# zju3dv/SMAP

Measured on NVIDIA H100. Metric: end-to-end FPS @832x512 (backbone+association+lift), higher is better.
Workload: dtype bf16x3 (split-bf16 operands, fp32 accumulate; fp32-faithful)

## Files before the change

### smap_b200/csrc/conv_tc.cuh

```cuda
#pragma once
#include <cuda.h>
#include "common.cuh"

namespace smapb {

struct alignas(64) ConvParams {
    CUtensorMap tmA;
    CUtensorMap tmA2;
    CUtensorMap tmB;
    CUtensorMap tmO;
    CUtensorMap tmR[3];
    int Hout, Wout, Nimg;
    int tw_log2, th;
    int tiles_x, tiles_y;
    int Cout;
    int kh, kw, stride, pad_y, pad_x;
    int kchunks;
    int kchunks2, stride2;
    int n_tiles;
    int total_tiles;
    const float* bias;
    int has_res;
    int n_post;
    __nv_bfloat16* out;
    float* out_f32;
    long long plane_stride;
    int relu;
    int reverse;
    int up_mode, up_Hi, up_Wi, up_pw, up_ph;
    long long* dbg;
    long long* dbg_tl;
    unsigned long long* sat;
};

// ... 196 lines not shown
    const uint32_t ring = (smem_u32(smem_raw) + 1024u + 1023u) & ~1023u;
    const uint32_t out_stage = ring + STAGES * Cfg::STAGE_BYTES;
    const uint32_t res_stage = out_stage + Cfg::OUT_BUFS * Cfg::SLOT_BYTES;

    const int warp = threadIdx.x >> 5;
    const int lane = threadIdx.x & 31;
    const bool tl = p.dbg_tl != nullptr && blockIdx.x == 0;
    if (tl && threadIdx.x == 0) p.dbg_tl[0] = clock64();
    const int n_extra = RING ? p.has_res + p.n_post : 0;
    const bool tma_out = p.out != nullptr;

    if (warp == 0 && lane == 0) {
        tma_prefetch_desc(&p.tmA);
        tma_prefetch_desc(&p.tmB);
        if (p.kchunks2) tma_prefetch_desc(&p.tmA2);
        if (tma_out) tma_prefetch_desc(&p.tmO);
        for (int e = 0; e < n_extra; e++) tma_prefetch_desc(&p.tmR[e]);
    }
    if (warp == 1 && lane == 0) {
        for (int s = 0; s < STAGES; s++) {
            mbar_init(&full_bar[s], 1);
            mbar_init(&empty_bar[s], 4);
        }
        for (int s = 0; s < Cfg::RES_BUFS; s++) {
            mbar_init(&rfull_bar[s], 1);
            mbar_init(&rempty_bar[s], 128);
        }
        fence_mbar_init();
    }
    __syncthreads();

// ... 135 lines not shown
                wgmma_wait<1>();
                if (prev_stage >= 0 && lane == 0) mbar_arrive(&empty_bar[prev_stage]);
                prev_stage = stage;
                if (++stage == STAGES) {
                    stage = 0;
                    phase ^= 1u;
                }
            }
            if (j + 1 < n_cta) turn_pass(TURN_MAIN, wg ^ 1);
            tally(ConvDbg::WAIT_FULL, w_full);
            wgmma_wait<0>();
            if (lane == 0) mbar_arrive(&empty_bar[prev_stage]);
            if (tl && leader && j == n_cta - 1) p.dbg_tl[3] = clock64();

            const long long t_epi0 = timed ? clock64() : 0;
            int py[4], px[4];
            bool valid[4];
            long long pix[4];
#pragma unroll
            for (int q = 0; q < 4; q++) {
                const int row = 64 * (q >> 1) + rw + 8 * (q & 1);
                py[q] = ty * p.th + (row >> p.tw_log2);
                px[q] = (tx << p.tw_log2) + (row & (tw - 1));
                valid[q] = (py[q] < p.Hout) && (px[q] < p.Wout) && (img < p.Nimg);
                pix[q] = ((long long)img * p.Hout + py[q]) * p.Wout + px[q];
            }
            auto row_of = [&](int q) { return 64 * (q >> 1) + rw + 8 * (q & 1); };
            const bool ring_turns = RING != 0 && n_extra > 0;
            if (ring_turns && j > 0) turn_wait(TURN_RING, wg);
            int rcnt = j * Cfg::CHUNKS * n_extra;
            auto ring_wait = [&]() -> uint32_t {
                const int m = rcnt++;
                const int rslot = m % Cfg::RES_DIV;
                tally(ConvDbg::WAIT_RING, mbar_wait_timed(&rfull_bar[rslot], (uint32_t)(m / Cfg::RES_DIV) & 1u, timed));
                return (uint32_t)rslot;
            };
            auto ring_release = [&](uint32_t rslot) {
                fence_proxy_async();
                mbar_arrive(&rempty_bar[rslot]);
            };
// ... 51 lines not shown
                                           (y1i - oy0) * p.up_pw + (x0i - ox0), (y1i - oy0) * p.up_pw + (x1i - ox0)};
#pragma unroll
                        for (int jj = 0; jj < 4; jj++) {
                            float2 s[4];
#pragma unroll
                            for (int k = 0; k < 4; k++) {
                                const uint32_t o = sw64_off(rr[k], jj) + 4 * q4;
                                s[k] = ring_f2(rb, o);
                            }
                            v[q][2 * jj] += hy0 * (wx0 * s[0].x + wx1 * s[1].x) + hy1 * (wx0 * s[2].x + wx1 * s[3].x);
                            v[q][2 * jj + 1] += hy0 * (wx0 * s[0].y + wx1 * s[1].y) + hy1 * (wx0 * s[2].y + wx1 * s[3].y);
                        }
                    }
                    ring_release(rslot);
                }
                if (p.relu) {
#pragma unroll
                    for (int q = 0; q < 4; q++)
#pragma unroll
                        for (int e = 0; e < 8; e++) v[q][e] = fmaxf(v[q][e], 0.f);
                }
                for (int e = 0; RING == 1 && e < p.n_post; e++) ring_add(v);
                if (tma_out) {
                    const uint32_t ob = ob0 + (uint32_t)((((j >> 1) * Cfg::CHUNKS + c) % Cfg::OUT_PER_WG) * Cfg::SLOT_BYTES);
                    if (leader) {
                        const long long t0 = timed ? clock64() : 0;
                        bulk_wait_read<Cfg::OUT_PER_WG - 1>();
                        tally(ConvDbg::WAIT_STAGE, timed ? clock64() - t0 : 0);
                    }
                    bool sat_warp = false;
                    if constexpr (E::F16) {
// ... 22 lines not shown
                                }
                            } else {
                                const uint32_t hw = E::pack2(a, b);
                                sts_u32(ob + o, hw);
                                if (NTERMS == 3)
                                    sts_u32(ob + Cfg::CHUNK_BYTES + o, E::pack2(a - E::lo(hw), b - E::hi(hw)));
                            }
                        }
                    if constexpr (E::F16)
                        if (sat_warp) saturation_add(p.sat, n_sat);
                    fence_proxy_async();
                    epi_bar_sync(wg);
                    if (leader) {
#pragma unroll
                        for (int t = 0; t < Cfg::TA; t++)
                            tma_store_5d(&p.tmO, ob + t * Cfg::CHUNK_BYTES, n0 + c0, tx << p.tw_log2, ty * p.th, img, t);
                        bulk_commit();
                    }
                } else {
#pragma unroll
                    for (int q = 0; q < 4; q++) {
                        if (!valid[q]) continue;
#pragma unroll
                        for (int jj = 0; jj < 4; jj++)
                            *reinterpret_cast<float2*>(p.out_f32 + pix[q] * p.Cout + n0 + c0 + 8 * jj + 2 * q4) =
                                make_float2(v[q][2 * jj], v[q][2 * jj + 1]);
                    }
                }
            }
            if (ring_turns && j + 1 < n_cta) turn_pass(TURN_RING, wg ^ 1);
            tally(ConvDbg::EPILOGUE, timed ? clock64() - t_epi0 : 0);
        }
        if (leader && tma_out) bulk_wait_all();
        if (leader && wg == ((n_cta - 1) & 1)) {
            if (p.dbg) {
                atomicAdd((unsigned long long*)&p.dbg[ConvDbg::TOTAL], (unsigned long long)(clock64() - t_begin));
                atomicAdd((unsigned long long*)&p.dbg[ConvDbg::CTAS], 1ull);
            }
            if (tl) p.dbg_tl[13] = p.dbg_tl[15] = clock64();
        }
// ... 5 lines not shown
```

### smap_b200/csrc/engine.h

```cpp
#pragma once
#include <cuda.h>
#include <cuda_runtime.h>
#include <stdint.h>
#include <stdlib.h>

#include <map>
#include <memory>
#include <string>
#include <vector>

#include "../../include/smap_b200.h"
#include "conv_tc.cuh"
#include "jpeg.h"
#include "png.h"
#include "preprocess.h"
#include "refine.h"

namespace smapb {

struct Act {
    __nv_bfloat16* ptr = nullptr;
    int N = 0, H = 0, W = 0, C = 0;
    long long plane() const { return (long long)N * H * W * C; }
};
struct ActF32 {
    float* ptr = nullptr;
    int N = 0, H = 0, W = 0, C = 0;
};

struct ConvLayer {
    std::string name;
    int Cin = 0, Cout = 0, Cout_pad = 0, k = 1, stride = 1, pad = 0;
    int Cin2 = 0, stride2 = 1;
    __nv_bfloat16* w_dev = nullptr;
    float* bias_dev = nullptr;
};

enum OpKind { OP_STEM, OP_S2D, OP_MAXPOOL, OP_CONV, OP_UPADD, OP_HEADMERGE, OP_TAPSUM };
struct Op {
    OpKind kind;
    ConvParams cp;
    int block_n = 0;
    double flops = 0;
    Act a, b, out;
    ActF32 f4, f3, f2;
    int cout = 0;
    int which_out = 0;
    const float* bias = nullptr;
    int stream = 0;
    std::vector<int> waits;
    bool record = false;
    cudaEvent_t ev = nullptr;
    std::string name;
    std::vector<const void*> inputs;
    int dims[4] = {0, 0, 0, 0};
};

struct Plan {
    int B = 0;
    std::vector<Op> ops;
    std::vector<void*> allocs;
    int n_conv = 0;
    double conv_flops = 0;
    std::map<const void*, int> producer;
    int last_side = -1;
};

}
// ... 145 lines not shown
```

### smap_b200/csrc/plan.cu

```cuda
#include <math.h>
#include <nvtx3/nvToolsExt.h>
#include <stdio.h>
#include <string.h>

#include <algorithm>
#include <mutex>

#include "../../include/smap_b200_debug.h"
#include "elementwise.h"
#include "engine.h"

using namespace smapb;

namespace {

std::mutex g_tiles_mu;
std::map<std::string, std::pair<int, int>> g_tiles;

inline uint16_t f32_to_bf16_rn(float f) {
    uint32_t u;
    memcpy(&u, &f, 4);
    if ((u & 0x7fffffffu) > 0x7f800000u) return (uint16_t)((u >> 16) | 0x40);
    const uint32_t lsb = (u >> 16) & 1u;
    u += 0x7fffu + lsb;
// ... 15 lines not shown
    if (!fn) {
        void* p = nullptr;
        cudaDriverEntryPointQueryResult qres;
        if (cudaGetDriverEntryPoint("cuTensorMapEncodeTiled", &p, cudaEnableDefault, &qres) == cudaSuccess &&
            qres == cudaDriverEntryPointSuccess)
            fn = reinterpret_cast<EncodeTiledFn>(p);
    }
    return fn;
}

struct ConvIO {
    const Act* in = nullptr;
    int relu = 0;
    const Act *in2 = nullptr, *res = nullptr, *post1 = nullptr, *post2 = nullptr, *up = nullptr, *out = nullptr;
    const ActF32* out_f32 = nullptr;
    std::vector<const void*> inputs() const {
        auto p = [](const Act* a) -> const void* { return a ? a->ptr : nullptr; };
        return {in->ptr, p(res), p(post1), p(post2), p(in2), p(up)};
    }
};
const char* const CONV_ROLES[6] = {"in", "res", "p1", "p2", "in2", "up"};

CUtensorMapDataType elem_dtype(const smapb_handle* h) { return h->f16 ? ElemF16::TMA_DTYPE : ElemBF16::TMA_DTYPE; }
int make_act_map(smapb_handle* h, CUtensorMap* m, const __nv_bfloat16* ptr, long long C, long long W, long long H,
                 long long N, int T, long long plane_elems, int box_w, int box_h, int stride, int box_c = 64) {
    EncodeTiledFn fn = get_encode_fn();
    if (!fn) return fail(h, -20, "cuTensorMapEncodeTiled entry point not available");
    cuuint64_t dims[5] = {(cuuint64_t)C, (cuuint64_t)W, (cuuint64_t)H, (cuuint64_t)N, (cuuint64_t)T};
    cuuint64_t strides[4] = {(cuuint64_t)C * 2, (cuuint64_t)W * C * 2, (cuuint64_t)H * W * C * 2,
                             (cuuint64_t)plane_elems * 2};
// ... 94 lines not shown
    return tw;
}

void set_tiling(ConvParams* cp, int nimg, int Hout, int Wout, int tw, int n_tiles) {
    const int th = 128 / tw;
    int twl = 0;
    while ((1 << twl) < tw) twl++;
    cp->Nimg = nimg;
    cp->Hout = Hout;
    cp->Wout = Wout;
    cp->tw_log2 = twl;
    cp->th = th;
    cp->tiles_x = (Wout + tw - 1) / tw;
    cp->tiles_y = (Hout + th - 1) / th;
    cp->n_tiles = n_tiles;
    cp->total_tiles = (int)((long long)cp->tiles_x * cp->tiles_y * nimg * n_tiles);
}

bool is_flat(const ConvLayer& L, const ConvIO& io) {
    return L.k == 1 && L.stride == 1 && (!io.in2 || L.stride2 == 1) && !io.up;
}
void conv_tiling(const ConvLayer& L, const ConvIO& io, int n_tiles, ConvParams* cp) {
    const Act& in = *io.in;
    const int Ho = (in.H + 2 * L.pad - L.k) / L.stride + 1, Wo = (in.W + 2 * L.pad - L.k) / L.stride + 1;
    if (is_flat(L, io))
        set_tiling(cp, 1, 1, (int)((long long)in.N * Ho * Wo), 128, n_tiles);
    else
        set_tiling(cp, in.N, Ho, Wo, patch_width(Ho, Wo, io.in2 ? std::max(L.stride, L.stride2) : L.stride, io.up),
                   n_tiles);
}

int setup_conv(smapb_handle* h, const ConvLayer& L, const ConvIO& io, int block_n, ConvParams* cp) {
    const Act& in = *io.in;
    const Act *in2 = io.in2, *res = io.res, *post1 = io.post1, *post2 = io.post2, *up = io.up;
    if (in.C != L.Cin) return fail(h, -30, "conv " + L.name + ": Cin mismatch");
    if (L.Cin % 64 != 0) return fail(h, -30, "conv " + L.name + ": Cin must be a multiple of 64");
    memset(cp, 0, sizeof(*cp));
    if ((L.Cin2 != 0) != (in2 != nullptr)) return fail(h, -30, "conv " + L.name + ": second input mismatch");
    if (L.Cin2 % 64 != 0) return fail(h, -30, "conv " + L.name + ": Cin2 must be a multiple of 64");
    if (in2 && (in2->C != L.Cin2 || L.k != 1 || L.stride != 1)) return fail(h, -30, "conv " + L.name + ": bad fused pair");
    if (up && (res || post1)) return fail(h, -30, "conv " + L.name + ": up-residual excludes other epilogue inputs");
    const bool flat = is_flat(L, io);
    conv_tiling(L, io, L.Cout_pad / block_n, cp);
    const int N = in.N, tw = 1 << cp->tw_log2, th = cp->th;
    auto a_map = [&](CUtensorMap* m, const Act& a, int s) {
        return flat ? make_act_map(h, m, a.ptr, a.C, cp->Wout, 1, 1, h->planes, a.plane(), 128, 1, 1)
                    : make_act_map(h, m, a.ptr, a.C, a.W, a.H, N, h->planes, a.plane(), tw * s, th * s, s);
    };
    int rc = a_map(&cp->tmA, in, L.stride);
    if (!rc && in2) rc = a_map(&cp->tmA2, *in2, L.stride2);
    if (rc) return rc;
    cp->Cout = L.Cout_pad;
    cp->kh = cp->kw = L.k;
    cp->stride = L.stride;
    cp->pad_y = cp->pad_x = L.pad;
    cp->kchunks = L.Cin / 64;
// ... 5 lines not shown
    if (up) {
        cp->up_mode = 1;
        cp->up_Hi = up->H;
        cp->up_Wi = up->W;
        cp->up_pw = tw / 2 + 2;
        cp->up_ph = th / 2 + 2;
        if (up->H * 2 != cp->Hout || up->W * 2 != cp->Wout || up->C != L.Cout_pad || cp->up_pw * cp->up_ph > 128)
            return fail(h, -30, "conv " + L.name + ": unsupported up-residual geometry");
        rc = make_act_map(h, &cp->tmR[0], up->ptr, up->C, up->W, up->H, N, h->planes, up->plane(), cp->up_pw,
                          cp->up_ph, 1, 32);
        if (rc) return rc;
    }
    if (post2 && !post1) return fail(h, -30, "conv " + L.name + ": post2 without post1");
    cp->out = io.out ? io.out->ptr : nullptr;
    cp->out_f32 = io.out_f32 ? io.out_f32->ptr : nullptr;
    cp->plane_stride = (long long)cp->Nimg * cp->Hout * cp->Wout * L.Cout_pad;
    cp->relu = io.relu;
    cp->sat = h->sat_dev;
    rc = make_w_map(h, &cp->tmB, L.w_dev, L.Cin + L.Cin2, L.Cout_pad, L.k * L.k, h->planes, block_n);
    if (rc) return rc;
    int n_in = up ? 1 : 0;
    for (const Act* t : {io.out, res, post1, post2}) {
        if (!t) continue;
        CUtensorMap* m = t == io.out ? &cp->tmO : &cp->tmR[n_in++];
        rc = make_act_map(h, m, t->ptr, L.Cout_pad, cp->Wout, cp->Hout, cp->Nimg, h->planes, t->plane(), tw, th, 1, 32);
        if (rc) return rc;
    }
    return 0;
}

int setup_stem_conv(smapb_handle* h, const __nv_bfloat16* s2d, long long s2d_plane, int N, int H2, int W2, const Act& out,
                    ConvParams* cp, int* block_n_out, double* flops_out) {
    const ConvLayer& L = h->stem_tc;
    memset(cp, 0, sizeof(*cp));
    EncodeTiledFn fn = get_encode_fn();
    if (!fn) return fail(h, -20, "cuTensorMapEncodeTiled entry point not available");
    set_tiling(cp, N, H2, W2, patch_width(H2, W2, 1, false), 1);
    const long long WP = W2 + 3;
    cuuint64_t dims[5] = {64, (cuuint64_t)W2, (cuuint64_t)H2, (cuuint64_t)N, (cuuint64_t)h->planes};
    cuuint64_t strides[4] = {32, (cuuint64_t)WP * 32, (cuuint64_t)H2 * WP * 32, (cuuint64_t)s2d_plane * 2};
// ... 1 lines not shown
    cuuint32_t es[5] = {1, 1, 1, 1, 1};
    CUresult r = fn(&cp->tmA, elem_dtype(h), 5, (void*)s2d, dims, strides, box, es,
                    CU_TENSOR_MAP_INTERLEAVE_NONE, CU_TENSOR_MAP_SWIZZLE_128B, CU_TENSOR_MAP_L2_PROMOTION_L2_256B,
                    CU_TENSOR_MAP_FLOAT_OOB_FILL_NONE);
    if (r != CUDA_SUCCESS) return fail(h, -22, "sliding-window tensor map rejected: " + std::to_string((int)r));
    cp->Cout = 64;
    cp->kh = 4, cp->kw = 1, cp->stride = 1, cp->pad_y = 2, cp->pad_x = 0;
    cp->kchunks = 1;
    cp->bias = L.bias_dev;
    cp->out = out.ptr;
    cp->plane_stride = out.plane();
    cp->relu = 1;
    cp->sat = h->sat_dev;
    int rc = make_w_map(h, &cp->tmB, L.w_dev, 64, 64, 4, h->planes, 64);
    if (rc) return rc;
    rc = make_act_map(h, &cp->tmO, out.ptr, 64, W2, H2, N, h->planes, out.plane(), 1 << cp->tw_log2, cp->th, 1, 32);
    if (rc) return rc;
    *block_n_out = 64;
    *flops_out = 2.0 * N * H2 * W2 * 64.0 * 147.0;
    return 0;
}

bool table_row_ok(const std::pair<int, int>& row) { return row.second == 1 && tile_shape_ok(row.first); }

int table_tile(smapb_handle* h, const ConvLayer& L, const ConvIO& io, int* bn) {
    const Act& in = *io.in;
    char key[256];
    snprintf(key, sizeof key, "%d/%d/%d k%d s%d %dx%dx%d r%d p%d u%d c2_%d s2_%d t%d%s", L.Cin, L.Cout_pad, L.Cin2, L.k,
             L.stride, in.N, in.H, in.W, io.res ? 1 : 0, (io.post1 ? 1 : 0) + (io.post2 ? 1 : 0), io.up ? 1 : 0, L.Cin2,
             L.stride2, h->nterms, h->f16 ? " f16" : "");
    {
        std::lock_guard<std::mutex> lk(g_tiles_mu);
        auto it = g_tiles.find(key);
        if (it != g_tiles.end() && table_row_ok(it->second)) {
            *bn = it->second.first;
            return 0;
        }
    }
    if (!h->autotune) return 0;
    cudaEvent_t e0, e1;
    cudaEventCreate(&e0);
    cudaEventCreate(&e1);
    float best_ms = 1e30f;
    int best = 0;
    for (int c : {128, 64, 32}) {
        if (L.Cout_pad % c) continue;
        if (c == 32 && L.Cout_pad > 64) continue;
        ConvParams trial;
        if (setup_conv(h, L, io, c, &trial)) continue;
        trial.sat = nullptr;
        float ms_best_c = 1e30f;
        for (int rep = 0; rep < 4; rep++) {
            cudaEventRecord(e0, nullptr);
            if (launch_conv(trial, c, h->nterms, h->f16, h->sm_count, nullptr, false) != cudaSuccess) {
                ms_best_c = 1e30f;
                break;
            }
            cudaEventRecord(e1, nullptr);
            if (cudaEventSynchronize(e1) != cudaSuccess) return fail(h, -10, "autotune launch failed");
            float ms = 0;
            cudaEventElapsedTime(&ms, e0, e1);
            if (rep > 0 && ms < ms_best_c) ms_best_c = ms;
        }
        if (ms_best_c < best_ms) best_ms = ms_best_c, best = c;
    }
    cudaEventDestroy(e0);
    cudaEventDestroy(e1);
    h->err.clear();
    if (!best) return 0;
    std::lock_guard<std::mutex> lk(g_tiles_mu);
    auto it = g_tiles.find(key);
    if (it == g_tiles.end() || !table_row_ok(it->second))
        g_tiles[key] = std::make_pair(best, 1);
    else
        best = it->second.first;
    *bn = best;
    return 0;
}

int choose_tile(smapb_handle* h, const ConvLayer& L, const ConvIO& io, bool tuned, int* bn_out) {
    ConvParams tiling;
    conv_tiling(L, io, 1, &tiling);
    const long long m_tiles = tiling.total_tiles;
    int bn = 0;
    const int num_kb = L.k * L.k * (L.Cin / 64) + L.Cin2 / 64;
    double best = 1e30;
    for (int c : {128, 64, 32}) {
        if (L.Cout_pad % c) continue;
        const double kb_cost = c == 128 ? 1.0 : c == 64 ? 0.6 : 0.4;
        const int n_extra = (io.res || io.up ? 1 : 0) + (io.post1 ? 1 : 0) + (io.post2 ? 1 : 0);
        const double epi = (c / 32) * (0.5 + 0.2 * n_extra + (io.up ? 0.5 : 0.0));
        const long long units = m_tiles * (L.Cout_pad / c);
        const double waves = (double)((units + h->sm_count - 1) / h->sm_count);
        double t = waves * (num_kb * kb_cost + epi);
        t *= (c == 64 ? 1.05 : c == 32 ? 1.10 : 1.0);
        if (t < best - 1e-9) best = t, bn = c;
    }
    if (!bn) return fail(h, -30, "conv " + L.name + ": no tile shape for Cout_pad " + std::to_string(L.Cout_pad));
    if (const char* force = getenv("SMAPB_FORCE_TILE")) {
        int fb = 0;
        if (sscanf(force, "%d", &fb) == 1 && tile_shape_ok(fb) && L.Cout_pad % fb == 0) bn = fb;
    }
    if (tuned) {
        const int rc = table_tile(h, L, io, &bn);
        if (rc) return rc;
    }
    *bn_out = bn;
    return 0;
}

int fold_unit(smapb_handle* h, const std::string& name, std::vector<float>* wf, std::vector<float>* bf, int* Cout,
              int* Cin, int* k) {
    auto need = [&](const char* suffix) -> const std::vector<float>* {
        auto it = h->raw.find(name + suffix);
        return it == h->raw.end() ? nullptr : &it->second;
    };
// ... 46 lines not shown
                if (h->planes == 2) host[plane + o] = f32_to_bf16_rn(v - bf16_to_f32(hi));
            }
    std::vector<float> bias(L.Cout_pad, 0.f);
    for (int co = 0; co < L.Cout; co++) bias[co] = bf[co];
    if (!L.w_dev) {
        if (dev_alloc(h, &L.w_dev, host.size())) return -10;
        if (dev_alloc(h, &L.bias_dev, bias.size())) return -10;
    }
    CK(cudaMemcpy(L.w_dev, host.data(), host.size() * 2, cudaMemcpyHostToDevice));
    CK(cudaMemcpy(L.bias_dev, bias.data(), bias.size() * 4, cudaMemcpyHostToDevice));
    return 0;
}

int pad32(int c) { return (c + 31) / 32 * 32; }

bool precision_ok(int p) { return p == SMAPB_PREC_BF16X3 || p == SMAPB_PREC_BF16 || p == SMAPB_PREC_FP16; }
void set_precision(smapb_handle* h, int precision) {
    h->nterms = precision == SMAPB_PREC_BF16X3 ? 3 : 1;
    h->planes = precision == SMAPB_PREC_BF16X3 ? 2 : 1;
    h->f16 = precision == SMAPB_PREC_FP16;
}

struct PlanBuilder {
    smapb_handle* h;
    Plan* plan;
    int rc = 0;
    int cur_stream = 0;

    void wire(const void* out_ptr, const std::vector<const void*>& inputs) {
        const int idx = (int)plan->ops.size() - 1;
// ... 68 lines not shown
        if (rc) return out;
        Op op;
        op.kind = OP_CONV;
        rc = choose_tile(h, *L, io, !f32, &op.block_n);
        if (!rc) rc = setup_conv(h, *L, io, op.block_n, &op.cp);
        op.flops = 2.0 * in.N * Ho * Wo * (double)L->Cout * (L->Cin * L->k * L->k + L->Cin2);
        op.name = name;
        op.cp.reverse = reverse_for(in.ptr);
        op.dims[0] = in.N, op.dims[1] = Ho, op.dims[2] = Wo, op.dims[3] = L->Cout_pad;
        plan->ops.push_back(op);
        wire(f32 ? (const void*)f32->ptr : out.ptr, io.inputs());
        plan->n_conv++;
        plan->conv_flops += op.flops;
        return out;
    }
};

const void* dumped_output(const smapb_handle* h, const Op& op, long long* bytes) {
    if (op.kind == OP_CONV && op.cp.out) return *bytes = op.cp.plane_stride * h->planes * 2, op.cp.out;
    if (op.kind == OP_CONV && op.cp.out_f32) return *bytes = op.cp.plane_stride * 4, op.cp.out_f32;
    if (op.out.ptr) return *bytes = op.out.plane() * h->planes * 2, op.out.ptr;
    *bytes = 0;
    return nullptr;
}

std::string debug_op_desc(const smapb_handle* h, const Op& op, const std::map<const void*, int>& dump_idx) {
    const bool is_conv = op.kind == OP_CONV;
    const bool stem_tc = is_conv && op.cp.kh == 4 && op.cp.kw == 1;
    const char* kind = is_conv ? (stem_tc ? "stem_tc" : op.cp.out ? "conv" : "conv_f32")
                       : op.kind == OP_STEM ? "stem" : op.kind == OP_S2D ? "s2d" : op.kind == OP_MAXPOOL ? "maxpool"
                       : op.kind == OP_UPADD ? "upadd" : "other";
    std::string s = "name=" + (op.name.empty() ? std::string("?") : op.name) + " kind=" + kind;
    if (op.kind == OP_STEM || op.kind == OP_S2D) s += " in=x";
    for (size_t r = 0; r < op.inputs.size(); r++) {
        if (!op.inputs[r]) continue;
        const char* role = is_conv ? (r < 6 ? CONV_ROLES[r] : "?") : (r == 0 ? "a" : "b");
        auto it = dump_idx.find(op.inputs[r]);
        s += std::string(" ") + role + "=" + (it == dump_idx.end() ? std::string("?") : std::to_string(it->second));
    }
    char buf[320];
    if (is_conv) {
        snprintf(buf, sizeof buf,
                 " tw=%d rev=%d k=%dx%d s=%d pad=%dx%d cin=%d cin2=%d s2=%d cout=%d out=%dx%dx%dx%d bn=%d relu=%d "
                 "hasres=%d post=%d upmode=%d tiles=%d nterms=%d",
                 1 << op.cp.tw_log2, op.cp.reverse, op.cp.kh, op.cp.kw, op.cp.stride, op.cp.pad_y, op.cp.pad_x,
                 op.cp.kchunks * 64, op.cp.kchunks2 * 64, op.cp.stride2, op.cp.Cout, op.dims[0], op.dims[1], op.dims[2],
                 op.dims[3], op.block_n, op.cp.relu, op.cp.has_res, op.cp.n_post, op.cp.up_mode, op.cp.total_tiles,
                 h->nterms);
    } else {
        snprintf(buf, sizeof buf, " out=%dx%dx%dx%d nterms=%d", op.out.N, op.out.H, op.out.W, op.out.C, h->nterms);
    }
    return s + buf + (h->f16 ? " dtype=f16" : "");
}

}

namespace smapb {

void free_plan(Plan* plan) {
    for (void* p : plan->allocs) cudaFree(p);
    for (Op& op : plan->ops)
        if (op.ev) cudaEventDestroy(op.ev);
    plan->allocs.clear();
// ... 65 lines not shown
            pb.wire(stem.ptr, {});
        }
    }
    Act x = pb.new_act(B, H / 4, W / 4, 64);
    {
        Op op;
        op.kind = OP_MAXPOOL;
        op.name = "top.maxpool";
        op.a = stem;
        op.out = x;
        plan->ops.push_back(op);
        pb.wire(x.ptr, {stem.ptr});
    }
    Act skip1[4], skip2[4];
    ActF32 res[4], resd3, resrd3;
    std::string name_d, name_rd;
    for (int s = 0; s < 3 && !pb.rc; s++) {
        const std::string pre = "stage" + std::to_string(s) + ".";
        const bool gen_skip = s != 2;
        Act feats[4];
        Act t = x;
        for (int li = 0; li < 4; li++) {
            for (int b = 0; b < LAYERS[li]; b++) {
                const std::string p = pre + "downsample.layer" + std::to_string(li + 1) + "." + std::to_string(b) + ".";
                Act o1 = pb.conv(p + "conv_bn_relu1", {&t, 1});
                Act o2 = pb.conv(p + "conv_bn_relu2", {&o1, 1});
                const bool last = (b == LAYERS[li] - 1) && s > 0;
                ConvIO c3{&o2, 1};
                if (b == 0 && !getenv("SMAPB_NO_FUSE_DS")) {
                    c3.in2 = &t;
                    t = pb.conv(p + "fused_conv3_downsample", c3);
                } else if (b == 0) {
                    Act idn = pb.conv(p + "downsample", {&t, 0});
                    c3.res = &idn;
                    t = pb.conv(p + "conv_bn_relu3", c3);
                } else {
                    c3.res = &t;
                    if (last) c3.post1 = &skip1[li], c3.post2 = &skip2[li];
                    t = pb.conv(p + "conv_bn_relu3", c3);
                }
            }
            feats[li] = t;
        }
        Act up_x;
        Act sk1[4], sk2[4];
        Act cross;
        for (int ind = 0; ind < 4 && !pb.rc; ind++) {
            const std::string p = pre + "upsample.up" + std::to_string(ind + 1) + ".";
            const Act& xin = feats[3 - ind];
            Act out;
            if (ind == 0) {
                out = pb.conv(p + "u_skip", {&xin, 1});
            } else {
                Act tl = pb.conv(p + "up_conv", {&up_x, 0});
                if (!getenv("SMAPB_NO_FUSE_UP")) {
                    ConvIO io{&xin, 1};
                    io.up = &tl;
                    out = pb.conv(p + "u_skip", io);
                } else {
                    Act a = pb.conv(p + "u_skip", {&xin, 0});
                    out = pb.new_act(a.N, a.H, a.W, a.C);
                    Op op;
                    op.kind = OP_UPADD;
                    op.a = a;
                    op.b = tl;
                    op.out = out;
                    plan->ops.push_back(op);
                    pb.wire(out.ptr, {a.ptr, tl.ptr});
                }
            }
            pb.cur_stream = h->two_streams ? 1 : 0;
            if (s == 2 && ind >= 1) {
                Act r1 = pb.conv(p + "res_conv1", {&out, 1});
                pb.conv(p + "res_conv2", {&r1, 0}, &res[ind]);
            }
            if (s == 2 && ind == 3) {
                Act d1 = pb.conv(p + "res_d_conv1", {&out, 1});
                pb.conv(p + "res_d_conv2.tapexp", {&d1, 0}, &resd3);
                Act rd1 = pb.conv(p + "res_rd_conv1", {&out, 1});
                pb.conv(p + "res_rd_conv2.tapexp", {&rd1, 0}, &resrd3);
                name_d = p + "res_d_conv2";
                name_rd = p + "res_rd_conv2";
            }
            if (gen_skip) {
                sk1[ind] = pb.conv(p + "skip1", {&xin, 1});
                sk2[ind] = pb.conv(p + "skip2", {&out, 1});
                pb.cur_stream = 0;
                if (ind == 3) cross = pb.conv(p + "cross_conv", {&out, 1});
            }
            pb.cur_stream = 0;
            up_x = out;
        }
        for (int li = 0; li < 4; li++) {
            skip1[li] = sk1[3 - li];
            skip2[li] = sk2[3 - li];
        }
        x = cross;
    }
    if (pb.rc) {
        free_plan(plan.get());
        return pb.rc;
    }
    {
// ... 117 lines not shown
        cudaDeviceSynchronize();
        for (auto& kv : h->plans) free_plan(kv.second.get());
        h->plans.clear();
        free_layers(h);
    }
    set_precision(h, precision);
    std::vector<std::string> units;
    for (auto& kv : h->raw) {
        const std::string& k = kv.first;
        const std::string suf = ".conv.weight";
        if (k.size() > suf.size() && k.compare(k.size() - suf.size(), suf.size(), suf) == 0)
            units.push_back(k.substr(0, k.size() - suf.size()));
    }
    if (units.empty()) return fail(h, -40, "no weights loaded");
    std::map<std::string, std::pair<std::vector<float>, std::vector<float>>> folded;
    for (const std::string& name : units) {
        std::vector<float> wf, bf;
        int Cout, Cin, k;
        int rc = fold_unit(h, name, &wf, &bf, &Cout, &Cin, &k);
        if (rc) return rc;
        if (name.find(".downsample.layer") != std::string::npos &&
            (name.find(".0.conv_bn_relu3") != std::string::npos ||
             (name.size() > 13 && name.compare(name.size() - 13, 13, ".0.downsample") == 0)))
            folded[name] = {wf, bf};
        if (name.find("res_d_conv2") != std::string::npos || name.find("res_rd_conv2") != std::string::npos)
            folded[name] = {wf, bf};
        if (name == "top.conv") {
            if (Cin != 3 || Cout != 64 || k != 7) return fail(h, -40, "top.conv must be 3->64 7x7");
            std::vector<float> w2(147 * 64);
            for (int co = 0; co < 64; co++)
                for (int ci = 0; ci < 3; ci++)
                    for (int ky = 0; ky < 7; ky++)
                        for (int kx = 0; kx < 7; kx++)
                            w2[((ky * 7 + kx) * 3 + ci) * 64 + co] = wf[((co * 3 + ci) * 7 + ky) * 7 + kx];
            if (!h->stem_w) {
// ... 78 lines not shown
        if (L0.k != 3) continue;
        ConvLayer& E = h->layers[nm + ".tapexp"];
        E.name = nm + ".tapexp";
        E.Cin = L0.Cin;
        E.Cout = 9 * L0.Cout;
        E.Cout_pad = pad32(E.Cout);
        E.k = 1, E.stride = 1, E.pad = 0;
        std::vector<float> wf((size_t)E.Cout * E.Cin), bf(E.Cout, 0.f);
        for (int c = 0; c < L0.Cout; c++)
            for (int ci = 0; ci < L0.Cin; ci++)
                for (int t = 0; t < 9; t++)
                    wf[(size_t)(t * L0.Cout + c) * E.Cin + ci] = kv.second.first[((size_t)c * L0.Cin + ci) * 9 + t];
        int rc4 = upload_conv_layer(h, E, 1, wf, bf);
        if (rc4) return rc4;
    }
    if (!h->stem_w) return fail(h, -40, "top.conv weights missing");
    h->finalized = true;
    return 0;
}

int smapb_set_tile_table(const char* text) {
    if (!text) return -1;
    std::lock_guard<std::mutex> lk(g_tiles_mu);
    int n = 0;
    const char* p = text;
    while (*p) {
        const char* e = strchr(p, '\n');
        std::string line = e ? std::string(p, e - p) : std::string(p);
        p = e ? e + 1 : p + line.size();
        if (line.empty() || line[0] == '#') continue;
// ... 21 lines not shown

__global__ void checksum_kernel(const uint32_t* __restrict__ p, long long nwords, unsigned long long* out) {
    unsigned long long acc = 0;
    for (long long i = (long long)blockIdx.x * blockDim.x + threadIdx.x; i < nwords; i += (long long)gridDim.x * blockDim.x)
        acc += (unsigned long long)p[i] * (unsigned long long)((i % 1021) + 1);
    atomicAdd(out, acc);
}
long long smapb_debug_dump(smapb_handle* h, int B, int idx, void* host, long long max_bytes, int which) {
    if (!h) return -1;
    cudaSetDevice(h->device);
    Plan* plan = nullptr;
    int rc = build_plan(h, B, &plan);
    if (rc) return rc;
    cudaDeviceSynchronize();
    int n = 0;
    for (const Op& op : plan->ops) {
        long long bytes = 0;
        const void* ptr = dumped_output(h, op, &bytes);
        if (!ptr) continue;
        if (n++ != idx) continue;
        (void)which;
        if (bytes > max_bytes) bytes = max_bytes;
        if (bytes > 0) CK(cudaMemcpy(host, ptr, (size_t)bytes, cudaMemcpyDefault));
        return bytes;
    }
    return -2;
}

int smapb_debug_checksums(smapb_handle* h, int B, unsigned long long* sums, int max_ops, char* desc, int desc_stride) {
    if (!h) return -1;
    cudaSetDevice(h->device);
    Plan* plan = nullptr;
    int rc = build_plan(h, B, &plan);
    if (rc) return rc;
    CK(cudaDeviceSynchronize());
    unsigned long long* d = nullptr;
    CK(cudaMalloc((void**)&d, 8));
    std::map<const void*, int> dump_idx;
    int n_dumped = 0;
    for (const Op& op : plan->ops) {
        long long bytes = 0;
        const void* out = dumped_output(h, op, &bytes);
        if (!out) continue;
        if (!dump_idx.emplace(out, n_dumped++).second) {
            cudaFree(d);
            return fail(h, -2, "smapb_debug_checksums: two ops share an output tensor (" + op.name + ")");
        }
    }
    int n = 0;
    for (const Op& op : plan->ops) {
        if (n >= max_ops) break;
        long long bytes = 0;
        const void* ptr = dumped_output(h, op, &bytes);
        if (!ptr) continue;
        const long long words = bytes / 4;
        CK(cudaMemset(d, 0, 8));
        checksum_kernel<<<132 * 4, 256>>>((const uint32_t*)ptr, words, d);
        CK(cudaMemcpy(&sums[n], d, 8, cudaMemcpyDeviceToHost));
        if (desc) snprintf(desc + (size_t)n * desc_stride, desc_stride, "%s", debug_op_desc(h, op, dump_idx).c_str());
        n++;
    }
    cudaFree(d);
    return n;
}

int smapb_plan_info(const smapb_handle* hc, int B, int* n_conv, double* conv_flops) {
    smapb_handle* h = const_cast<smapb_handle*>(hc);
    if (!h) return -1;
    if (!h->finalized) return fail(h, -2, "weights not finalized");
    cudaSetDevice(h->device);
    Plan* plan = nullptr;
    int rc = build_plan(h, B, &plan);
    if (rc) return rc;
    if (n_conv) *n_conv = plan->n_conv;
    if (conv_flops) *conv_flops = plan->conv_flops;
    return 0;
// ... 198 lines not shown
```

Before: 480.0.

## Merge sibling 1x1 convs sharing an input into one multi-output GEMM

Concatenates the weights of sibling 1x1 convolutions that read the same activation (skip2+up_conv, res_conv1+up_conv, the three res conv1 branches) into one merged layer. The kernel picks a per-segment output tensor map and relu bit from the N-tile index, so one launch writes several separate outputs. This cuts kernel launches and re-reads of the shared input, and gives each launch more N-tiles to fill the GPU. In exchange it adds per-segment bookkeeping in the epilogue, requires the block width to divide every segment, and restructures stream placement and the debug dump paths.

```diff
diff --git a/smap_b200/csrc/conv_tc.cuh b/smap_b200/csrc/conv_tc.cuh
--- a/smap_b200/csrc/conv_tc.cuh
+++ b/smap_b200/csrc/conv_tc.cuh
@@ -3,12 +3,14 @@
 #include "common.cuh"
 
 namespace smapb {
+
+constexpr int SEG_MAX = 3;
 
 struct alignas(64) ConvParams {
     CUtensorMap tmA;
     CUtensorMap tmA2;
     CUtensorMap tmB;
-    CUtensorMap tmO;
+    CUtensorMap tmO[SEG_MAX];
     CUtensorMap tmR[3];
     int Hout, Wout, Nimg;
     int tw_log2, th;
@@ -18,6 +20,7 @@
     int kchunks;
     int kchunks2, stride2;
     int n_tiles;
+    int seg_nt[SEG_MAX];
     int total_tiles;
     const float* bias;
     int has_res;
@@ -244,7 +247,8 @@
         tma_prefetch_desc(&p.tmA);
         tma_prefetch_desc(&p.tmB);
         if (p.kchunks2) tma_prefetch_desc(&p.tmA2);
-        if (tma_out) tma_prefetch_desc(&p.tmO);
+        if (tma_out) tma_prefetch_desc(&p.tmO[0]);
+        for (int s = 1; RING == 0 && s < SEG_MAX && p.seg_nt[s] < p.n_tiles; s++) tma_prefetch_desc(&p.tmO[s]);
         for (int e = 0; e < n_extra; e++) tma_prefetch_desc(&p.tmR[e]);
     }
     if (warp == 1 && lane == 0) {
@@ -410,16 +414,16 @@
             if (tl && leader && j == n_cta - 1) p.dbg_tl[3] = clock64();
 
             const long long t_epi0 = timed ? clock64() : 0;
+            const int seg = RING ? 0 : (n0 >= p.seg_nt[1] * BLOCK_N) + (n0 >= p.seg_nt[2] * BLOCK_N);
+            const int n0_out = RING ? n0 : n0 - p.seg_nt[seg] * BLOCK_N;
             int py[4], px[4];
             bool valid[4];
-            long long pix[4];
 #pragma unroll
             for (int q = 0; q < 4; q++) {
                 const int row = 64 * (q >> 1) + rw + 8 * (q & 1);
                 py[q] = ty * p.th + (row >> p.tw_log2);
                 px[q] = (tx << p.tw_log2) + (row & (tw - 1));
                 valid[q] = (py[q] < p.Hout) && (px[q] < p.Wout) && (img < p.Nimg);
-                pix[q] = ((long long)img * p.Hout + py[q]) * p.Wout + px[q];
             }
             auto row_of = [&](int q) { return 64 * (q >> 1) + rw + 8 * (q & 1); };
             const bool ring_turns = RING != 0 && n_extra > 0;
@@ -501,7 +505,7 @@
                     }
                     ring_release(rslot);
                 }
-                if (p.relu) {
+                if (RING ? p.relu : (p.relu >> seg) & 1) {
 #pragma unroll
                     for (int q = 0; q < 4; q++)
 #pragma unroll
@@ -554,16 +558,18 @@
                     if (leader) {
 #pragma unroll
                         for (int t = 0; t < Cfg::TA; t++)
-                            tma_store_5d(&p.tmO, ob + t * Cfg::CHUNK_BYTES, n0 + c0, tx << p.tw_log2, ty * p.th, img, t);
+                            tma_store_5d(&p.tmO[seg], ob + t * Cfg::CHUNK_BYTES, n0_out + c0, tx << p.tw_log2, ty * p.th,
+                                         img, t);
                         bulk_commit();
                     }
                 } else {
 #pragma unroll
                     for (int q = 0; q < 4; q++) {
                         if (!valid[q]) continue;
+                        const long long pix = ((long long)img * p.Hout + py[q]) * p.Wout + px[q];
 #pragma unroll
                         for (int jj = 0; jj < 4; jj++)
-                            *reinterpret_cast<float2*>(p.out_f32 + pix[q] * p.Cout + n0 + c0 + 8 * jj + 2 * q4) =
+                            *reinterpret_cast<float2*>(p.out_f32 + pix * p.Cout + n0 + c0 + 8 * jj + 2 * q4) =
                                 make_float2(v[q][2 * jj], v[q][2 * jj + 1]);
                     }
                 }
diff --git a/smap_b200/csrc/engine.h b/smap_b200/csrc/engine.h
--- a/smap_b200/csrc/engine.h
+++ b/smap_b200/csrc/engine.h
@@ -28,10 +28,16 @@
     int N = 0, H = 0, W = 0, C = 0;
 };
 
+struct ConvSeg {
+    std::string name;
+    int Cout = 0, Cout_pad = 0;
+};
+
 struct ConvLayer {
     std::string name;
     int Cin = 0, Cout = 0, Cout_pad = 0, k = 1, stride = 1, pad = 0;
     int Cin2 = 0, stride2 = 1;
+    std::vector<ConvSeg> segs;
     __nv_bfloat16* w_dev = nullptr;
     float* bias_dev = nullptr;
 };
@@ -52,6 +58,8 @@
     bool record = false;
     cudaEvent_t ev = nullptr;
     std::string name;
+    std::vector<ConvSeg> segs;
+    std::vector<Act> seg_out;
     std::vector<const void*> inputs;
     int dims[4] = {0, 0, 0, 0};
 };
diff --git a/smap_b200/csrc/plan.cu b/smap_b200/csrc/plan.cu
--- a/smap_b200/csrc/plan.cu
+++ b/smap_b200/csrc/plan.cu
@@ -53,6 +53,7 @@
     int relu = 0;
     const Act *in2 = nullptr, *res = nullptr, *post1 = nullptr, *post2 = nullptr, *up = nullptr, *out = nullptr;
     const ActF32* out_f32 = nullptr;
+    const Act* seg_out[SEG_MAX - 1] = {nullptr, nullptr};
     std::vector<const void*> inputs() const {
         auto p = [](const Act* a) -> const void* { return a ? a->ptr : nullptr; };
         return {in->ptr, p(res), p(post1), p(post2), p(in2), p(up)};
@@ -177,6 +178,7 @@
     cp->tiles_x = (Wout + tw - 1) / tw;
     cp->tiles_y = (Hout + th - 1) / th;
     cp->n_tiles = n_tiles;
+    for (int s = 1; s < SEG_MAX; s++) cp->seg_nt[s] = n_tiles;
     cp->total_tiles = (int)((long long)cp->tiles_x * cp->tiles_y * nimg * n_tiles);
 }
 
@@ -191,6 +193,13 @@
     else
         set_tiling(cp, in.N, Ho, Wo, patch_width(Ho, Wo, io.in2 ? std::max(L.stride, L.stride2) : L.stride, io.up),
                    n_tiles);
+}
+
+int seg_cout_pad(const ConvLayer& L, int s) { return L.segs.empty() ? L.Cout_pad : L.segs[s].Cout_pad; }
+bool tile_fits(const ConvLayer& L, int bn) {
+    for (size_t s = 0; s < std::max<size_t>(L.segs.size(), 1); s++)
+        if (seg_cout_pad(L, (int)s) % bn) return false;
+    return true;
 }
 
 int setup_conv(smapb_handle* h, const ConvLayer& L, const ConvIO& io, int block_n, ConvParams* cp) {
@@ -203,6 +212,12 @@
     if (L.Cin2 % 64 != 0) return fail(h, -30, "conv " + L.name + ": Cin2 must be a multiple of 64");
     if (in2 && (in2->C != L.Cin2 || L.k != 1 || L.stride != 1)) return fail(h, -30, "conv " + L.name + ": bad fused pair");
     if (up && (res || post1)) return fail(h, -30, "conv " + L.name + ": up-residual excludes other epilogue inputs");
+    const int n_seg = L.segs.empty() ? 1 : (int)L.segs.size();
+    if (n_seg > 1) {
+        bool ok = n_seg <= SEG_MAX && io.out && !in2 && !res && !post1 && !up && tile_fits(L, block_n);
+        for (int s = 1; ok && s < n_seg; s++) ok = io.seg_out[s - 1] != nullptr;
+        if (!ok) return fail(h, -30, "conv " + L.name + ": bad merged layer");
+    }
     const bool flat = is_flat(L, io);
     conv_tiling(L, io, L.Cout_pad / block_n, cp);
     const int N = in.N, tw = 1 << cp->tw_log2, th = cp->th;
@@ -238,7 +253,7 @@
     if (post2 && !post1) return fail(h, -30, "conv " + L.name + ": post2 without post1");
     cp->out = io.out ? io.out->ptr : nullptr;
     cp->out_f32 = io.out_f32 ? io.out_f32->ptr : nullptr;
-    cp->plane_stride = (long long)cp->Nimg * cp->Hout * cp->Wout * L.Cout_pad;
+    cp->plane_stride = (long long)cp->Nimg * cp->Hout * cp->Wout * seg_cout_pad(L, 0);
     cp->relu = io.relu;
     cp->sat = h->sat_dev;
     rc = make_w_map(h, &cp->tmB, L.w_dev, L.Cin + L.Cin2, L.Cout_pad, L.k * L.k, h->planes, block_n);
@@ -246,8 +261,16 @@
     int n_in = up ? 1 : 0;
     for (const Act* t : {io.out, res, post1, post2}) {
         if (!t) continue;
-        CUtensorMap* m = t == io.out ? &cp->tmO : &cp->tmR[n_in++];
-        rc = make_act_map(h, m, t->ptr, L.Cout_pad, cp->Wout, cp->Hout, cp->Nimg, h->planes, t->plane(), tw, th, 1, 32);
+        CUtensorMap* m = t == io.out ? &cp->tmO[0] : &cp->tmR[n_in++];
+        rc = make_act_map(h, m, t->ptr, seg_cout_pad(L, 0), cp->Wout, cp->Hout, cp->Nimg, h->planes, t->plane(), tw, th, 1,
+                          32);
+        if (rc) return rc;
+    }
+    for (int s = 1; s < n_seg; s++) {
+        const Act& t = *io.seg_out[s - 1];
+        cp->seg_nt[s] = cp->seg_nt[s - 1] + seg_cout_pad(L, s - 1) / block_n;
+        rc = make_act_map(h, &cp->tmO[s], t.ptr, seg_cout_pad(L, s), cp->Wout, cp->Hout, cp->Nimg, h->planes, t.plane(), tw,
+                          th, 1, 32);
         if (rc) return rc;
     }
     return 0;
@@ -279,25 +302,29 @@
     cp->sat = h->sat_dev;
     int rc = make_w_map(h, &cp->tmB, L.w_dev, 64, 64, 4, h->planes, 64);
     if (rc) return rc;
-    rc = make_act_map(h, &cp->tmO, out.ptr, 64, W2, H2, N, h->planes, out.plane(), 1 << cp->tw_log2, cp->th, 1, 32);
+    rc = make_act_map(h, &cp->tmO[0], out.ptr, 64, W2, H2, N, h->planes, out.plane(), 1 << cp->tw_log2, cp->th, 1, 32);
     if (rc) return rc;
     *block_n_out = 64;
     *flops_out = 2.0 * N * H2 * W2 * 64.0 * 147.0;
     return 0;
 }
 
-bool table_row_ok(const std::pair<int, int>& row) { return row.second == 1 && tile_shape_ok(row.first); }
+bool table_row_ok(const ConvLayer& L, const std::pair<int, int>& row) {
+    return row.second == 1 && tile_shape_ok(row.first) && tile_fits(L, row.first);
+}
 
 int table_tile(smapb_handle* h, const ConvLayer& L, const ConvIO& io, int* bn) {
     const Act& in = *io.in;
     char key[256];
-    snprintf(key, sizeof key, "%d/%d/%d k%d s%d %dx%dx%d r%d p%d u%d c2_%d s2_%d t%d%s", L.Cin, L.Cout_pad, L.Cin2, L.k,
+    std::string segs;
+    for (size_t s = 0; s < L.segs.size(); s++) segs += (s ? "+" : " m") + std::to_string(L.segs[s].Cout_pad);
+    snprintf(key, sizeof key, "%d/%d/%d k%d s%d %dx%dx%d r%d p%d u%d c2_%d s2_%d t%d%s%s", L.Cin, L.Cout_pad, L.Cin2, L.k,
              L.stride, in.N, in.H, in.W, io.res ? 1 : 0, (io.post1 ? 1 : 0) + (io.post2 ? 1 : 0), io.up ? 1 : 0, L.Cin2,
-             L.stride2, h->nterms, h->f16 ? " f16" : "");
+             L.stride2, h->nterms, segs.c_str(), h->f16 ? " f16" : "");
     {
         std::lock_guard<std::mutex> lk(g_tiles_mu);
         auto it = g_tiles.find(key);
-        if (it != g_tiles.end() && table_row_ok(it->second)) {
+        if (it != g_tiles.end() && table_row_ok(L, it->second)) {
             *bn = it->second.first;
             return 0;
         }
@@ -309,7 +336,7 @@
     float best_ms = 1e30f;
     int best = 0;
     for (int c : {128, 64, 32}) {
-        if (L.Cout_pad % c) continue;
+        if (!tile_fits(L, c)) continue;
         if (c == 32 && L.Cout_pad > 64) continue;
         ConvParams trial;
         if (setup_conv(h, L, io, c, &trial)) continue;
@@ -335,7 +362,7 @@
     if (!best) return 0;
     std::lock_guard<std::mutex> lk(g_tiles_mu);
     auto it = g_tiles.find(key);
-    if (it == g_tiles.end() || !table_row_ok(it->second))
+    if (it == g_tiles.end() || !table_row_ok(L, it->second))
         g_tiles[key] = std::make_pair(best, 1);
     else
         best = it->second.first;
@@ -351,7 +378,7 @@
     const int num_kb = L.k * L.k * (L.Cin / 64) + L.Cin2 / 64;
     double best = 1e30;
     for (int c : {128, 64, 32}) {
-        if (L.Cout_pad % c) continue;
+        if (!tile_fits(L, c)) continue;
         const double kb_cost = c == 128 ? 1.0 : c == 64 ? 0.6 : 0.4;
         const int n_extra = (io.res || io.up ? 1 : 0) + (io.post1 ? 1 : 0) + (io.post2 ? 1 : 0);
         const double epi = (c / 32) * (0.5 + 0.2 * n_extra + (io.up ? 0.5 : 0.0));
@@ -364,7 +391,7 @@
     if (!bn) return fail(h, -30, "conv " + L.name + ": no tile shape for Cout_pad " + std::to_string(L.Cout_pad));
     if (const char* force = getenv("SMAPB_FORCE_TILE")) {
         int fb = 0;
-        if (sscanf(force, "%d", &fb) == 1 && tile_shape_ok(fb) && L.Cout_pad % fb == 0) bn = fb;
+        if (sscanf(force, "%d", &fb) == 1 && tile_shape_ok(fb) && tile_fits(L, fb)) bn = fb;
     }
     if (tuned) {
         const int rc = table_tile(h, L, io, &bn);
@@ -441,6 +468,29 @@
 
 int pad32(int c) { return (c + 31) / 32 * 32; }
 
+std::string merged_name(const std::vector<std::string>& names) {
+    std::string n;
+    for (const std::string& u : names) n += (n.empty() ? "" : "+") + u;
+    return n;
+}
+std::string up_unit(int stage, int ind, const char* unit) {
+    return "stage" + std::to_string(stage) + ".upsample.up" + std::to_string(ind + 1) + "." + unit;
+}
+std::vector<std::string> sibling_group(int stage, int ind) {
+    if (stage < 2)
+        return {up_unit(stage, ind, "skip2"), ind < 3 ? up_unit(stage, ind + 1, "up_conv") : up_unit(stage, 3, "cross_conv")};
+    if (ind == 0) return {};
+    if (ind < 3) return {up_unit(2, ind, "res_conv1"), up_unit(2, ind + 1, "up_conv")};
+    return {up_unit(2, 3, "res_conv1"), up_unit(2, 3, "res_d_conv1"), up_unit(2, 3, "res_rd_conv1")};
+}
+std::vector<std::vector<std::string>> sibling_groups() {
+    std::vector<std::vector<std::string>> g;
+    for (int stage = 0; stage < 3; stage++)
+        for (int ind = 0; ind < 4; ind++)
+            if (!sibling_group(stage, ind).empty()) g.push_back(sibling_group(stage, ind));
+    return g;
+}
+
 bool precision_ok(int p) { return p == SMAPB_PREC_BF16X3 || p == SMAPB_PREC_BF16 || p == SMAPB_PREC_FP16; }
 void set_precision(smapb_handle* h, int precision) {
     h->nterms = precision == SMAPB_PREC_BF16X3 ? 3 : 1;
@@ -539,39 +589,79 @@
         plan->conv_flops += op.flops;
         return out;
     }
+    std::vector<Act> siblings(const std::vector<std::string>& names, ConvIO io) {
+        std::vector<Act> outs(names.size());
+        if (rc) return outs;
+        const ConvLayer* L = layer(merged_name(names));
+        if (!L) return outs;
+        const Act& in = *io.in;
+        for (size_t s = 0; s < names.size(); s++) {
+            outs[s] = new_act(in.N, in.H, in.W, L->segs[s].Cout_pad);
+            if (s) io.seg_out[s - 1] = &outs[s];
+        }
+        io.out = &outs[0];
+        if (rc) return outs;
+        Op op;
+        op.kind = OP_CONV;
+        rc = choose_tile(h, *L, io, true, &op.block_n);
+        if (!rc) rc = setup_conv(h, *L, io, op.block_n, &op.cp);
+        for (const ConvSeg& g : L->segs) op.flops += 2.0 * in.N * in.H * in.W * (double)g.Cout * L->Cin;
+        op.name = L->name;
+        op.segs = L->segs;
+        op.seg_out = outs;
+        op.cp.reverse = reverse_for(in.ptr);
+        op.dims[0] = in.N, op.dims[1] = in.H, op.dims[2] = in.W, op.dims[3] = L->Cout_pad;
+        plan->ops.push_back(op);
+        wire(outs[0].ptr, io.inputs());
+        for (size_t s = 1; s < outs.size(); s++) plan->producer[outs[s].ptr] = (int)plan->ops.size() - 1;
+        plan->n_conv++;
+        plan->conv_flops += op.flops;
+        return outs;
+    }
 };
 
-const void* dumped_output(const smapb_handle* h, const Op& op, long long* bytes) {
-    if (op.kind == OP_CONV && op.cp.out) return *bytes = op.cp.plane_stride * h->planes * 2, op.cp.out;
-    if (op.kind == OP_CONV && op.cp.out_f32) return *bytes = op.cp.plane_stride * 4, op.cp.out_f32;
-    if (op.out.ptr) return *bytes = op.out.plane() * h->planes * 2, op.out.ptr;
-    *bytes = 0;
-    return nullptr;
-}
-
-std::string debug_op_desc(const smapb_handle* h, const Op& op, const std::map<const void*, int>& dump_idx) {
+struct Dumped {
+    const void* ptr;
+    long long bytes;
+    int seg;
+};
+std::vector<Dumped> dumped_outputs(const smapb_handle* h, const Op& op) {
+    std::vector<Dumped> d;
+    for (size_t s = 0; s < op.seg_out.size(); s++)
+        d.push_back({op.seg_out[s].ptr, op.seg_out[s].plane() * h->planes * 2, (int)s});
+    if (!op.seg_out.empty()) return d;
+    if (op.kind == OP_CONV && op.cp.out) d.push_back({op.cp.out, op.cp.plane_stride * h->planes * 2, -1});
+    else if (op.kind == OP_CONV && op.cp.out_f32) d.push_back({op.cp.out_f32, op.cp.plane_stride * 4, -1});
+    else if (op.out.ptr) d.push_back({op.out.ptr, op.out.plane() * h->planes * 2, -1});
+    return d;
+}
+
+std::string debug_op_desc(const smapb_handle* h, const Op& op, int seg, const std::map<const void*, int>& dump_idx) {
     const bool is_conv = op.kind == OP_CONV;
     const bool stem_tc = is_conv && op.cp.kh == 4 && op.cp.kw == 1;
     const char* kind = is_conv ? (stem_tc ? "stem_tc" : op.cp.out ? "conv" : "conv_f32")
                        : op.kind == OP_STEM ? "stem" : op.kind == OP_S2D ? "s2d" : op.kind == OP_MAXPOOL ? "maxpool"
                        : op.kind == OP_UPADD ? "upadd" : "other";
-    std::string s = "name=" + (op.name.empty() ? std::string("?") : op.name) + " kind=" + kind;
+    const std::string& name = seg >= 0 ? op.segs[seg].name : op.name;
+    std::string s = "name=" + (name.empty() ? std::string("?") : name) + " kind=" + kind;
     if (op.kind == OP_STEM || op.kind == OP_S2D) s += " in=x";
+    const bool seg_inputs = seg <= 0;
     for (size_t r = 0; r < op.inputs.size(); r++) {
-        if (!op.inputs[r]) continue;
+        if (!op.inputs[r] || (r > 0 && !seg_inputs)) continue;
         const char* role = is_conv ? (r < 6 ? CONV_ROLES[r] : "?") : (r == 0 ? "a" : "b");
         auto it = dump_idx.find(op.inputs[r]);
         s += std::string(" ") + role + "=" + (it == dump_idx.end() ? std::string("?") : std::to_string(it->second));
     }
     char buf[320];
     if (is_conv) {
+        int dims[4] = {op.dims[0], op.dims[1], op.dims[2], seg >= 0 ? op.segs[seg].Cout_pad : op.dims[3]};
         snprintf(buf, sizeof buf,
                  " tw=%d rev=%d k=%dx%d s=%d pad=%dx%d cin=%d cin2=%d s2=%d cout=%d out=%dx%dx%dx%d bn=%d relu=%d "
                  "hasres=%d post=%d upmode=%d tiles=%d nterms=%d",
                  1 << op.cp.tw_log2, op.cp.reverse, op.cp.kh, op.cp.kw, op.cp.stride, op.cp.pad_y, op.cp.pad_x,
-                 op.cp.kchunks * 64, op.cp.kchunks2 * 64, op.cp.stride2, op.cp.Cout, op.dims[0], op.dims[1], op.dims[2],
-                 op.dims[3], op.block_n, op.cp.relu, op.cp.has_res, op.cp.n_post, op.cp.up_mode, op.cp.total_tiles,
-                 h->nterms);
+                 op.cp.kchunks * 64, op.cp.kchunks2 * 64, op.cp.stride2, dims[3], dims[0], dims[1], dims[2], dims[3],
+                 op.block_n, (op.cp.relu >> std::max(seg, 0)) & 1, seg_inputs ? op.cp.has_res : 0,
+                 seg_inputs ? op.cp.n_post : 0, seg_inputs ? op.cp.up_mode : 0, op.cp.total_tiles, h->nterms);
     } else {
         snprintf(buf, sizeof buf, " out=%dx%dx%dx%d nterms=%d", op.out.N, op.out.H, op.out.W, op.out.C, h->nterms);
     }
@@ -667,6 +757,7 @@
     }
     Act skip1[4], skip2[4];
     ActF32 res[4], resd3, resrd3;
+    const bool fuse_sib = !getenv("SMAPB_NO_FUSE_SIBLINGS");
     std::string name_d, name_rd;
     for (int s = 0; s < 3 && !pb.rc; s++) {
         const std::string pre = "stage" + std::to_string(s) + ".";
@@ -696,16 +787,20 @@
             feats[li] = t;
         }
         Act up_x;
+        Act up_t;
         Act sk1[4], sk2[4];
         Act cross;
         for (int ind = 0; ind < 4 && !pb.rc; ind++) {
             const std::string p = pre + "upsample.up" + std::to_string(ind + 1) + ".";
             const Act& xin = feats[3 - ind];
             Act out;
+            const std::vector<std::string> group_out = fuse_sib ? sibling_group(s, ind) : std::vector<std::string>();
+            Act tl = up_t;
+            if (ind > 0 && !tl.ptr) tl = pb.conv(p + "up_conv", {&up_x, 0});
+            up_t = Act();
             if (ind == 0) {
                 out = pb.conv(p + "u_skip", {&xin, 1});
             } else {
-                Act tl = pb.conv(p + "up_conv", {&up_x, 0});
                 if (!getenv("SMAPB_NO_FUSE_UP")) {
                     ConvIO io{&xin, 1};
                     io.up = &tl;
@@ -722,24 +817,31 @@
                     pb.wire(out.ptr, {a.ptr, tl.ptr});
                 }
             }
-            pb.cur_stream = h->two_streams ? 1 : 0;
+            const int side = h->two_streams ? 1 : 0;
+            std::vector<Act> m;
+            if (!group_out.empty()) {
+                pb.cur_stream = group_out.size() == 3 ? side : 0;
+                m = pb.siblings(group_out, {&out, group_out.size() == 3 ? 0b111 : s < 2 && ind == 3 ? 0b11 : 0b01});
+                if (ind < 3) up_t = m[1];
+            }
+            pb.cur_stream = side;
             if (s == 2 && ind >= 1) {
-                Act r1 = pb.conv(p + "res_conv1", {&out, 1});
+                Act r1 = m.empty() ? pb.conv(p + "res_conv1", {&out, 1}) : m[0];
                 pb.conv(p + "res_conv2", {&r1, 0}, &res[ind]);
             }
             if (s == 2 && ind == 3) {
-                Act d1 = pb.conv(p + "res_d_conv1", {&out, 1});
+                Act d1 = m.empty() ? pb.conv(p + "res_d_conv1", {&out, 1}) : m[1];
                 pb.conv(p + "res_d_conv2.tapexp", {&d1, 0}, &resd3);
-                Act rd1 = pb.conv(p + "res_rd_conv1", {&out, 1});
+                Act rd1 = m.empty() ? pb.conv(p + "res_rd_conv1", {&out, 1}) : m[2];
                 pb.conv(p + "res_rd_conv2.tapexp", {&rd1, 0}, &resrd3);
                 name_d = p + "res_d_conv2";
                 name_rd = p + "res_rd_conv2";
             }
             if (gen_skip) {
                 sk1[ind] = pb.conv(p + "skip1", {&xin, 1});
-                sk2[ind] = pb.conv(p + "skip2", {&out, 1});
+                sk2[ind] = m.empty() ? pb.conv(p + "skip2", {&out, 1}) : m[0];
                 pb.cur_stream = 0;
-                if (ind == 3) cross = pb.conv(p + "cross_conv", {&out, 1});
+                if (ind == 3) cross = m.empty() ? pb.conv(p + "cross_conv", {&out, 1}) : m[1];
             }
             pb.cur_stream = 0;
             up_x = out;
@@ -887,11 +989,15 @@
     }
     if (units.empty()) return fail(h, -40, "no weights loaded");
     std::map<std::string, std::pair<std::vector<float>, std::vector<float>>> folded;
+    std::map<std::string, std::pair<std::vector<float>, std::vector<float>>> sib_folded;
+    const std::vector<std::vector<std::string>> groups = sibling_groups();
     for (const std::string& name : units) {
         std::vector<float> wf, bf;
         int Cout, Cin, k;
         int rc = fold_unit(h, name, &wf, &bf, &Cout, &Cin, &k);
         if (rc) return rc;
+        for (const auto& g : groups)
+            if (std::find(g.begin(), g.end(), name) != g.end()) sib_folded[name] = {wf, bf};
         if (name.find(".downsample.layer") != std::string::npos &&
             (name.find(".0.conv_bn_relu3") != std::string::npos ||
              (name.size() > 13 && name.compare(name.size() - 13, 13, ".0.downsample") == 0)))
@@ -1000,6 +1106,35 @@
         int rc4 = upload_conv_layer(h, E, 1, wf, bf);
         if (rc4) return rc4;
     }
+    for (const auto& g : groups) {
+        bool all = true;
+        for (const std::string& u : g) all = all && sib_folded.count(u);
+        if (!all) continue;
+        ConvLayer& M = h->layers[merged_name(g)];
+        M.name = merged_name(g);
+        M.segs.clear();
+        M.Cin = h->layers[g[0]].Cin;
+        M.Cout_pad = 0;
+        for (const std::string& u : g) {
+            const ConvLayer& U = h->layers[u];
+            if (U.k != 1 || U.stride != 1 || U.Cin != M.Cin)
+                return fail(h, -40, "sibling unit " + u + " is not a 1x1 conv over the input of " + g[0]);
+            M.segs.push_back({u, U.Cout, U.Cout_pad});
+            M.Cout_pad += U.Cout_pad;
+        }
+        M.Cout = M.Cout_pad;
+        M.k = 1, M.stride = 1, M.pad = 0;
+        std::vector<float> wf((size_t)M.Cout * M.Cin, 0.f), bf(M.Cout, 0.f);
+        int row = 0;
+        for (const ConvSeg& sg : M.segs) {
+            const auto& f = sib_folded[sg.name];
+            std::copy(f.first.begin(), f.first.end(), wf.begin() + (size_t)row * M.Cin);
+            std::copy(f.second.begin(), f.second.end(), bf.begin() + row);
+            row += sg.Cout_pad;
+        }
+        int rc5 = upload_conv_layer(h, M, 1, wf, bf);
+        if (rc5) return rc5;
+    }
     if (!h->stem_w) return fail(h, -40, "top.conv weights missing");
     h->finalized = true;
     return 0;
@@ -1051,16 +1186,14 @@
     if (rc) return rc;
     cudaDeviceSynchronize();
     int n = 0;
-    for (const Op& op : plan->ops) {
-        long long bytes = 0;
-        const void* ptr = dumped_output(h, op, &bytes);
-        if (!ptr) continue;
-        if (n++ != idx) continue;
-        (void)which;
-        if (bytes > max_bytes) bytes = max_bytes;
-        if (bytes > 0) CK(cudaMemcpy(host, ptr, (size_t)bytes, cudaMemcpyDefault));
-        return bytes;
-    }
+    for (const Op& op : plan->ops)
+        for (const Dumped& d : dumped_outputs(h, op)) {
+            if (n++ != idx) continue;
+            (void)which;
+            const long long bytes = std::min(d.bytes, max_bytes);
+            if (bytes > 0) CK(cudaMemcpy(host, d.ptr, (size_t)bytes, cudaMemcpyDefault));
+            return bytes;
+        }
     return -2;
 }
 
@@ -1075,28 +1208,23 @@
     CK(cudaMalloc((void**)&d, 8));
     std::map<const void*, int> dump_idx;
     int n_dumped = 0;
-    for (const Op& op : plan->ops) {
-        long long bytes = 0;
-        const void* out = dumped_output(h, op, &bytes);
-        if (!out) continue;
-        if (!dump_idx.emplace(out, n_dumped++).second) {
-            cudaFree(d);
-            return fail(h, -2, "smapb_debug_checksums: two ops share an output tensor (" + op.name + ")");
-        }
-    }
+    for (const Op& op : plan->ops)
+        for (const Dumped& o : dumped_outputs(h, op))
+            if (!dump_idx.emplace(o.ptr, n_dumped++).second) {
+                cudaFree(d);
+                return fail(h, -2, "smapb_debug_checksums: two ops share an output tensor (" + op.name + ")");
+            }
     int n = 0;
-    for (const Op& op : plan->ops) {
-        if (n >= max_ops) break;
-        long long bytes = 0;
-        const void* ptr = dumped_output(h, op, &bytes);
-        if (!ptr) continue;
-        const long long words = bytes / 4;
-        CK(cudaMemset(d, 0, 8));
-        checksum_kernel<<<132 * 4, 256>>>((const uint32_t*)ptr, words, d);
-        CK(cudaMemcpy(&sums[n], d, 8, cudaMemcpyDeviceToHost));
-        if (desc) snprintf(desc + (size_t)n * desc_stride, desc_stride, "%s", debug_op_desc(h, op, dump_idx).c_str());
-        n++;
-    }
+    for (const Op& op : plan->ops)
+        for (const Dumped& o : dumped_outputs(h, op)) {
+            if (n >= max_ops) break;
+            CK(cudaMemset(d, 0, 8));
+            checksum_kernel<<<132 * 4, 256>>>((const uint32_t*)o.ptr, o.bytes / 4, d);
+            CK(cudaMemcpy(&sums[n], d, 8, cudaMemcpyDeviceToHost));
+            if (desc)
+                snprintf(desc + (size_t)n * desc_stride, desc_stride, "%s", debug_op_desc(h, op, o.seg, dump_idx).c_str());
+            n++;
+        }
     cudaFree(d);
     return n;
 }
```

Measured after the change: 484.1 (median of 6 runs). Within noise of the previous version (+0.8%).
